# timoklein/alphazero-gym

Measured on NVIDIA B200. Metric: MCTS simulations/sec (batched trees), higher is better.
Workload: dtype f64 tree statistics + env dynamics / f32 network with exact int8-sliced tensor-core products

## Files before the change

### alphazero_gym_b200/csrc/engine.cu

```cuda
#include <cuda_runtime.h>

#include <cmath>
#include <cstdio>
#include <cstdlib>
#include <cstring>
#include <initializer_list>
#include <map>
#include <string>
#include <tuple>
#include <utility>
#include <vector>

#include "../../include/azg.h"
#include "common.cuh"
#include "env.cuh"
#include "mlp.cuh"
#include "qmlp.cuh"
#include "qmlp2.cuh"
#include "search_wg.cuh"
#include "selfplay.cuh"
#include "tree_continuous.cuh"
#include "tree_discrete.cuh"

static thread_local std::string g_err;
// ... 713 lines not shown
            if (ce != cudaSuccess || ee != cudaSuccess) {
                if (g) cudaGraphDestroy(g);
                return fail(AZG_ECUDA, std::string("graph capture: ") + cudaGetErrorString(ce != cudaSuccess ? ce : ee));
            }
            cudaGraphExec_t ge = nullptr;
            cudaError_t ie = cudaGraphInstantiate(&ge, g, 0);
            cudaGraphDestroy(g);
            if (ie != cudaSuccess) return fail(AZG_ECUDA, std::string("graph instantiate: ") + cudaGetErrorString(ie));
            if (e->graphs.size() > 32) {
                for (auto& kv : e->graphs) cudaGraphExecDestroy(kv.second);
                e->graphs.clear();
            }
            e->graphs[key] = ge;
            e->launches = n;
            it = e->graphs.find(key);
        }
        e->launches = 2 * (int64_t)N + 3 + (e->cfg.variant == AZG_CONTINUOUS ? 1 : 0) - (tape ? N + 1 : 0);
        if (e->tree_word != tree_id0) {
            k_set_seed<<<1, 1, 0, st>>>(e->d_seed + 1, (uint64_t)tree_id0);
            CK(cudaGetLastError());
            e->tree_word = tree_id0;
        }
        CK(cudaGraphLaunch(it->second, st));
    }
    e->last_B = B;
    e->last_N = N;
    return AZG_OK;
}

extern "C" int azg_search_discrete(azg_engine* e, int32_t B, const double* d_root_state, const int32_t* d_root_n_init,
                                   int32_t n_rollouts, int64_t tree_id0, void* stream) {
    if (e && e->cfg.variant != AZG_DISCRETE) return fail(AZG_EINVAL, "engine was created for the continuous variant");
    return run_search(e, B, d_root_state, d_root_n_init, n_rollouts, tree_id0, (cudaStream_t)stream);
}

extern "C" int azg_search_continuous(azg_engine* e, int32_t B, const double* d_root_state, int32_t n_rollouts, int64_t tree_id0,
                                     void* stream) {
    if (e && e->cfg.variant != AZG_CONTINUOUS) return fail(AZG_EINVAL, "engine was created for the discrete variant");
    return run_search(e, B, d_root_state, nullptr, n_rollouts, tree_id0, (cudaStream_t)stream);
}

extern "C" int azg_profile_search(azg_engine* e, int32_t B, const double* d_root_state, const int32_t* d_root_n_init,
                                  int32_t n_rollouts, int64_t tree_id0, void* stream, float ms_out[3], int32_t launches_out[3]) {
    if (!e || !d_root_state || !ms_out || !launches_out) return fail(AZG_EINVAL, "null argument");
    if (B < 1 || B > e->cfg.max_trees) return fail(AZG_EINVAL, "B out of range");
    if (n_rollouts < 1 || n_rollouts > e->cfg.max_rollouts) return fail(AZG_EINVAL, "n_rollouts out of range");
    if (!e->weights_set && !e->tapeV) return fail(AZG_EINVAL, "azg_set_weights has not been called");
    CK(cudaSetDevice(e->cfg.device));
    cudaStream_t st = (cudaStream_t)stream;
    const int sd = e->cfg.variant == AZG_DISCRETE ? 4 : 2;
    if (d_root_state != e->root_state)
        CK(cudaMemcpyAsync(e->root_state, d_root_state, (size_t)B * sd * sizeof(double), cudaMemcpyDeviceToDevice, st));
    if (e->cfg.variant == AZG_DISCRETE) {
        if (d_root_n_init) CK(cudaMemcpyAsync(e->root_n_init, d_root_n_init, (size_t)B * sizeof(int32_t), cudaMemcpyDeviceToDevice, st));
        else CK(cudaMemsetAsync(e->root_n_init, 0, (size_t)B * sizeof(int32_t), st));
    }
    Prof prof;
    cudaError_t ce = cudaSuccess;
    e->launches = enqueue_search(e, B, n_rollouts, tree_id0, st, &ce, &prof);
    cudaError_t se = cudaStreamSynchronize(st);
    for (int k = 0; k < 3; ++k) { ms_out[k] = 0.0f; launches_out[k] = 0; }
    for (size_t i = 0; i < prof.cls.size(); ++i) {
        float ms = 0.0f;
        if (cudaEventElapsedTime(&ms, prof.ev[2 * i], prof.ev[2 * i + 1]) == cudaSuccess) {
            ms_out[prof.cls[i]] += ms;
            launches_out[prof.cls[i]] += 1;
        }
    }
    for (cudaEvent_t ev : prof.ev) cudaEventDestroy(ev);
    if (ce != cudaSuccess) return fail(AZG_ECUDA, std::string("kernel launch: ") + cudaGetErrorString(ce));
    if (se != cudaSuccess) return fail(AZG_ECUDA, std::string("sync: ") + cudaGetErrorString(se));
    e->last_B = B;
    e->last_N = n_rollouts;
    return AZG_OK;
}

extern "C" int azg_root_results(azg_engine* e, int32_t B, float* d_actions, int32_t* d_counts, double* d_Q, double* d_V_target,
                                int32_t* d_n_children, void* stream) {
    if (!e || !d_actions || !d_counts || !d_Q || !d_V_target || !d_n_children) return fail(AZG_EINVAL, "null argument");
    if (B < 1 || B > e->cfg.max_trees) return fail(AZG_EINVAL, "B out of range");
    CK(cudaSetDevice(e->cfg.device));
    cudaStream_t st = (cudaStream_t)stream;
    const TreeParams p = make_params(e, B, 0);
    const int tb = 128, tg = (B + tb - 1) / tb;
    if (e->cfg.variant == AZG_DISCRETE) k_results_discrete<<<tg, tb, 0, st>>>(p, e->cmax, d_actions, d_counts, d_Q, d_V_target, d_n_children);
    else k_results_continuous<<<tg, tb, 0, st>>>(p, e->cmax, d_actions, d_counts, d_Q, d_V_target, d_n_children);
    CK(cudaGetLastError());
    return AZG_OK;
}

extern "C" int azg_status(azg_engine* e, void* stream) {
    if (!e) return fail(AZG_EINVAL, "null engine");
    CK(cudaSetDevice(e->cfg.device));
    int32_t h = 0;
    CK(cudaMemcpyAsync(&h, e->err, sizeof h, cudaMemcpyDeviceToHost, (cudaStream_t)stream));
    CK(cudaStreamSynchronize((cudaStream_t)stream));
    if (h) CK(cudaMemsetAsync(e->err, 0, sizeof h, (cudaStream_t)stream));
    if (h & ERR_NAN) return fail(AZG_ENAN, "NaN in a UCT vector (helpers.py:47-48)");
    if (h & ERR_CAPACITY) return fail(AZG_ECAPACITY, "tree arena or child fan-out capacity exceeded");
    return AZG_OK;
}

extern "C" int azg_search_host(azg_engine* e, int32_t B, const double* h_root_state, const int32_t* h_root_n_init, int32_t n_rollouts,
                               int64_t tree_id0, float* h_actions, int32_t* h_counts, double* h_Q, double* h_V_target,
                               int32_t* h_n_children) {
    if (!e || !h_root_state || !h_actions || !h_counts || !h_Q || !h_V_target || !h_n_children) return fail(AZG_EINVAL, "null argument");
    if (B < 1 || B > e->cfg.max_trees) return fail(AZG_EINVAL, "B out of range");
    if (e->cfg.variant == AZG_CONTINUOUS && h_root_n_init) return fail(AZG_EINVAL, "root_n_init is a discrete-only argument");
    CK(cudaSetDevice(e->cfg.device));
    cudaStream_t st = e->own_stream;
    const int sd = e->cfg.variant == AZG_DISCRETE ? 4 : 2;
    const size_t cm = e->cmax;
    char* hp = (char*)e->h_pinned;
    double* p_root = (double*)hp; hp += (size_t)B * 4 * sizeof(double);
    double* p_Q = (double*)hp; hp += (size_t)B * cm * sizeof(double);
    double* p_Vt = (double*)hp; hp += (size_t)B * sizeof(double);
    float* p_act = (float*)hp; hp += (size_t)B * cm * sizeof(float);
    int32_t* p_cnt = (int32_t*)hp; hp += (size_t)B * cm * sizeof(int32_t);
    int32_t* p_nc = (int32_t*)hp; hp += (size_t)B * sizeof(int32_t);
    int32_t* p_rn = (int32_t*)hp;
    {
        cudaPointerAttributes at;
        const bool root_pinned = cudaPointerGetAttributes(&at, h_root_state) == cudaSuccess && at.type == cudaMemoryTypeHost;
        cudaGetLastError();
        if (!root_pinned) memcpy(p_root, h_root_state, (size_t)B * sd * sizeof(double));
        CK(cudaMemcpyAsync(e->root_state, root_pinned ? h_root_state : p_root, (size_t)B * sd * sizeof(double), cudaMemcpyHostToDevice, st));
    }
    const int32_t* d_rn = nullptr;
    if (h_root_n_init) {
        memcpy(p_rn, h_root_n_init, (size_t)B * sizeof(int32_t));
        CK(cudaMemcpyAsync(e->root_n_init, p_rn, (size_t)B * sizeof(int32_t), cudaMemcpyHostToDevice, st));
        d_rn = e->root_n_init;
    }
    int rc = run_search(e, B, e->root_state, d_rn, n_rollouts, tree_id0, st);
    if (rc) return rc;
    rc = azg_root_results(e, B, e->r_actions, e->r_counts, e->r_Q, e->r_Vt, e->r_nchild, st);
    if (rc) return rc;
    auto pinned = [](const void* h) {
        cudaPointerAttributes at;
        const bool ok = cudaPointerGetAttributes(&at, h) == cudaSuccess && at.type == cudaMemoryTypeHost;
        cudaGetLastError();
        return ok;
    };
    const bool direct = pinned(h_actions) && pinned(h_counts) && pinned(h_Q) && pinned(h_V_target) && pinned(h_n_children);
    CK(cudaMemcpyAsync(direct ? h_actions : p_act, e->r_actions, (size_t)B * cm * sizeof(float), cudaMemcpyDeviceToHost, st));
    CK(cudaMemcpyAsync(direct ? h_counts : p_cnt, e->r_counts, (size_t)B * cm * sizeof(int32_t), cudaMemcpyDeviceToHost, st));
    CK(cudaMemcpyAsync(direct ? h_Q : p_Q, e->r_Q, (size_t)B * cm * sizeof(double), cudaMemcpyDeviceToHost, st));
    CK(cudaMemcpyAsync(direct ? h_V_target : p_Vt, e->r_Vt, (size_t)B * sizeof(double), cudaMemcpyDeviceToHost, st));
    CK(cudaMemcpyAsync(direct ? h_n_children : p_nc, e->r_nchild, (size_t)B * sizeof(int32_t), cudaMemcpyDeviceToHost, st));
    rc = azg_status(e, st);
    if (!direct) {
        memcpy(h_actions, p_act, (size_t)B * cm * sizeof(float));
        memcpy(h_counts, p_cnt, (size_t)B * cm * sizeof(int32_t));
        memcpy(h_Q, p_Q, (size_t)B * cm * sizeof(double));
        memcpy(h_V_target, p_Vt, (size_t)B * sizeof(double));
        memcpy(h_n_children, p_nc, (size_t)B * sizeof(int32_t));
    }
    return rc;
}

extern "C" int azg_search_host_begin(azg_engine* e, int32_t slot, int32_t B, const double* h_root_state, const int32_t* h_root_n_init,
                                     int32_t n_rollouts, int64_t tree_id0, float* h_actions, int32_t* h_counts, double* h_Q,
                                     double* h_V_target, int32_t* h_n_children) {
    if (!e || !h_root_state || !h_actions || !h_counts || !h_Q || !h_V_target || !h_n_children) return fail(AZG_EINVAL, "null argument");
    if (slot < 0 || slot > 1) return fail(AZG_EINVAL, "slot must be 0 or 1");
    if (B < 1 || B > e->cfg.max_trees) return fail(AZG_EINVAL, "B out of range");
    if (e->cfg.variant == AZG_CONTINUOUS && h_root_n_init) return fail(AZG_EINVAL, "root_n_init is a discrete-only argument");
    if (e->pending[slot]) return fail(AZG_EINVAL, "slot is still in flight: call azg_search_host_end first");
    CK(cudaSetDevice(e->cfg.device));
    auto pinned = [](const void* h) {
        cudaPointerAttributes at;
        const bool ok = cudaPointerGetAttributes(&at, h) == cudaSuccess && at.type == cudaMemoryTypeHost;
        cudaGetLastError();
        return ok;
    };
    if (!(pinned(h_root_state) && pinned(h_actions) && pinned(h_counts) && pinned(h_Q) && pinned(h_V_target) && pinned(h_n_children) &&
          (!h_root_n_init || pinned(h_root_n_init))))
        return fail(AZG_EINVAL, "azg_search_host_begin needs page-locked host buffers (cudaHostAlloc / cudaHostRegister / pin_memory)");
    const size_t cm = e->cmax, Bm = e->cfg.max_trees;
    if (!e->copy_stream) {
        CK(cudaStreamCreateWithFlags(&e->copy_stream, cudaStreamNonBlocking));
        for (int k = 0; k < 2; ++k) {
            CK(cudaEventCreateWithFlags(&e->ev_done[k], cudaEventDisableTiming));
            CK(cudaEventCreateWithFlags(&e->ev_copied[k], cudaEventDisableTiming));
        }
        CK(cudaMallocHost(&e->h_err, 2 * sizeof(int32_t)));
        CK(cudaMalloc(&e->r2_actions, Bm * cm * sizeof(float)));
        CK(cudaMalloc(&e->r2_counts, Bm * cm * sizeof(int32_t)));
        CK(cudaMalloc(&e->r2_Q, Bm * cm * sizeof(double)));
        CK(cudaMalloc(&e->r2_Vt, Bm * sizeof(double)));
        CK(cudaMalloc(&e->r2_nchild, Bm * sizeof(int32_t)));
    }
    float* ra = slot ? e->r2_actions : e->r_actions;
    int32_t* rc_ = slot ? e->r2_counts : e->r_counts;
    double* rq = slot ? e->r2_Q : e->r_Q;
    double* rv = slot ? e->r2_Vt : e->r_Vt;
    int32_t* rn = slot ? e->r2_nchild : e->r_nchild;
    cudaStream_t st = e->own_stream;
    const int sd = e->cfg.variant == AZG_DISCRETE ? 4 : 2;
    CK(cudaMemcpyAsync(e->root_state, h_root_state, (size_t)B * sd * sizeof(double), cudaMemcpyHostToDevice, st));
    const int32_t* d_rn = nullptr;
    if (h_root_n_init) {
        CK(cudaMemcpyAsync(e->root_n_init, h_root_n_init, (size_t)B * sizeof(int32_t), cudaMemcpyHostToDevice, st));
        d_rn = e->root_n_init;
    }
    int rc = run_search(e, B, e->root_state, d_rn, n_rollouts, tree_id0, st);
    if (rc) return rc;
    rc = azg_root_results(e, B, ra, rc_, rq, rv, rn, st);
    if (rc) return rc;
    CK(cudaMemcpyAsync(e->h_err + slot, e->err, sizeof(int32_t), cudaMemcpyDeviceToHost, st));
    CK(cudaMemsetAsync(e->err, 0, sizeof(int32_t), st));
    CK(cudaEventRecord(e->ev_done[slot], st));
    CK(cudaStreamWaitEvent(e->copy_stream, e->ev_done[slot], 0));
    CK(cudaMemcpyAsync(h_actions, ra, (size_t)B * cm * sizeof(float), cudaMemcpyDeviceToHost, e->copy_stream));
    CK(cudaMemcpyAsync(h_counts, rc_, (size_t)B * cm * sizeof(int32_t), cudaMemcpyDeviceToHost, e->copy_stream));
    CK(cudaMemcpyAsync(h_Q, rq, (size_t)B * cm * sizeof(double), cudaMemcpyDeviceToHost, e->copy_stream));
    CK(cudaMemcpyAsync(h_V_target, rv, (size_t)B * sizeof(double), cudaMemcpyDeviceToHost, e->copy_stream));
    CK(cudaMemcpyAsync(h_n_children, rn, (size_t)B * sizeof(int32_t), cudaMemcpyDeviceToHost, e->copy_stream));
    CK(cudaEventRecord(e->ev_copied[slot], e->copy_stream));
    e->pending[slot] = true;
    return AZG_OK;
}

extern "C" int azg_search_host_end(azg_engine* e, int32_t slot) {
    if (!e || slot < 0 || slot > 1) return fail(AZG_EINVAL, "bad argument");
    if (!e->pending[slot]) return fail(AZG_EINVAL, "nothing in flight in this slot");
    CK(cudaSetDevice(e->cfg.device));
    CK(cudaEventSynchronize(e->ev_copied[slot]));
    e->pending[slot] = false;
    const int32_t h = e->h_err[slot];
    if (h & ERR_NAN) return fail(AZG_ENAN, "NaN in a UCT vector (helpers.py:47-48)");
    if (h & ERR_CAPACITY) return fail(AZG_ECAPACITY, "tree arena or child fan-out capacity exceeded");
    return AZG_OK;
}

static cudaError_t fetch_ctl(const azg_engine* e, int B, std::vector<CCtl>& out) {
    const size_t BS = e->cfg.max_trees;
    std::vector<uint4> plane(B);
    out.resize(B);
    for (int k = 0; k < 4; ++k) {
        cudaError_t ce = cudaMemcpy(plane.data(), e->ctl + k * BS, (size_t)B * sizeof(uint4), cudaMemcpyDeviceToHost);
        if (ce != cudaSuccess) return ce;
        for (int t = 0; t < B; ++t) reinterpret_cast<uint4*>(&out[t])[k] = plane[t];
    }
    return cudaSuccess;
}
static cudaError_t fetch_et(const azg_engine* e, int B, std::vector<CHot>& out) {
    const size_t BS = e->cfg.max_trees;
    std::vector<CHot> plane(B);
    out.resize((size_t)B * CROOT_MAX_KIDS);
    for (int j = 0; j < CROOT_MAX_KIDS; ++j) {
        cudaError_t ce = cudaMemcpy(plane.data(), e->et + j * BS, (size_t)B * sizeof(CHot), cudaMemcpyDeviceToHost);
        if (ce != cudaSuccess) return ce;
        for (int t = 0; t < B; ++t) out[(size_t)t * CROOT_MAX_KIDS + j] = plane[t];
    }
    return cudaSuccess;
}

extern "C" int azg_get_counters(azg_engine* e, int32_t B, int64_t out[8]) {
    if (!e || !out) return fail(AZG_EINVAL, "null argument");
    if (B < 1 || B > e->cfg.max_trees) return fail(AZG_EINVAL, "B out of range");
    CK(cudaSetDevice(e->cfg.device));
    CK(cudaDeviceSynchronize());
    std::vector<uint32_t> c(4 * (size_t)B);
    std::vector<int32_t> dr(B, 0), pw(B, 0);
    const int LB = e->last_B > 0 ? e->last_B : B;
    std::vector<uint32_t> all(4 * (size_t)LB);
    CK(cudaMemcpy(all.data(), e->ctr, all.size() * sizeof(uint32_t), cudaMemcpyDeviceToHost));
    if (e->cfg.variant == AZG_DISCRETE) {
        CK(cudaMemcpy(dr.data(), e->draws, (size_t)B * sizeof(int32_t), cudaMemcpyDeviceToHost));
    } else {
        std::vector<CCtl> cc;
        CK(fetch_ctl(e, B, cc));
        for (int t = 0; t < B; ++t) { dr[t] = cc[t].draws; pw[t] = cc[t].pw; }
    }
    for (int k = 0; k < 8; ++k) out[k] = 0;
    const int nb = std::min(B, LB);
    for (int t = 0; t < nb; ++t) {
        out[1] += all[t];
        out[2] += all[(size_t)LB + t];
        out[6] += all[(size_t)2 * LB + t];
        out[4] += all[(size_t)3 * LB + t];
        out[5] += dr[t];
        out[3] += pw[t];
    }
    out[0] = (int64_t)nb * e->last_N;
    out[7] = e->launches;
    return AZG_OK;
}

extern "C" int azg_fused_stats(azg_engine* e, int64_t out[8]) {
    if (!e || !out) return fail(AZG_EINVAL, "null argument");
    CK(cudaSetDevice(e->cfg.device));
    CK(cudaDeviceSynchronize());
    unsigned long long h[16];
    CK(cudaMemcpy(h, e->stats, sizeof h, cudaMemcpyDeviceToHost));
    CK(cudaMemset(e->stats, 0, sizeof h));
#ifdef AZG_TREE_PROF
    fprintf(stderr, "tree step sections (cycles summed over warps): load %llu backup %llu select %llu insert %llu expand+store %llu | per-WG total %llu over %llu warpgroups | "
            "discrete level loop: scores %llu draw+pick %llu next row %llu over %llu warp-levels\n", h[8], h[9], h[10], h[11], h[12], h[0], h[4], h[13], h[14], h[11], h[15]);
#endif
#ifdef AZG_EVAL_PROF
    if (e->last_fused_kind == 2)
        fprintf(stderr, "k_search_wg, cycles per warpgroup and search spent waiting for MMAs: at column step 0 of a layer %llu | step 1 %llu | steps 2..7 %llu | kernel %llu\n",
                h[8] / (h[4] ? h[4] : 1), h[9] / (h[4] ? h[4] : 1), h[10] / (h[4] ? h[4] : 1), h[0] / (h[4] ? h[4] : 1));
    else
    fprintf(stderr, "evaluation timeline of epilogue thread 0, cycles per CTA and search: layer 0 %llu | MMA wait %llu | load + convert %llu | stash / quantise / heads %llu | "
            "post-processing wait %llu | tree phase %llu | kernel %llu\n", h[8] / (h[4] ? h[4] : 1), h[9] / (h[4] ? h[4] : 1), h[10] / (h[4] ? h[4] : 1), h[11] / (h[4] ? h[4] : 1),
            h[12] / (h[4] ? h[4] : 1), h[13] / (h[4] ? h[4] : 1), h[0] / (h[4] ? h[4] : 1));
#endif
    for (int k = 0; k < 8; ++k) out[k] = (int64_t)h[k];
    out[5] = e->last_fused_kind;
    return AZG_OK;
}

extern "C" int azg_set_seed(azg_engine* e, uint64_t seed, void* stream) {
    if (!e) return fail(AZG_EINVAL, "null engine");
    CK(cudaSetDevice(e->cfg.device));
    k_set_seed<<<1, 1, 0, (cudaStream_t)stream>>>(e->d_seed, seed);
    CK(cudaGetLastError());
    e->cfg.seed = seed;
    return AZG_OK;
}

extern "C" int azg_set_reward_model(azg_engine* e, double reward_step, double reward_terminal) {
    if (!e) return fail(AZG_EINVAL, "null engine");
    if (!(reward_step == reward_step) || !(reward_terminal == reward_terminal) || std::isinf(reward_step) || std::isinf(reward_terminal))
        return fail(AZG_EINVAL, "rewards must be finite");
    if (e->cfg.variant != AZG_DISCRETE && (reward_step != 1.0 || reward_terminal != 1.0))
        return fail(AZG_EINVAL, "the reward model applies to the discrete (CartPole) search");
    if (reward_step == e->reward_step && reward_terminal == e->reward_terminal) return AZG_OK;
    CK(cudaSetDevice(e->cfg.device));
    CK(cudaDeviceSynchronize());
    for (auto& kv : e->graphs) cudaGraphExecDestroy(kv.second);
    e->graphs.clear();
    e->reward_step = reward_step; e->reward_terminal = reward_terminal;
    return AZG_OK;
}

extern "C" uint64_t azg_selfplay_seed(uint64_t seed, int64_t step_index) { return seed + (uint64_t)step_index * 0x9E3779B97F4A7C15ull; }

extern "C" int azg_selfplay_step(azg_engine* e, int32_t B, const azg_selfplay_io* io, int32_t n_rollouts, int64_t tree_id0,
                                 int64_t step_index, uint64_t base_seed, int32_t max_episode_length, int32_t deterministic,
                                 int32_t by_value, double temperature, void* stream) {
    if (!e || !io) return fail(AZG_EINVAL, "null argument");
    if (!io->d_env_state || !io->d_ep_step || !io->d_episode || !io->d_obs || !io->d_actions || !io->d_counts || !io->d_Q ||
        !io->d_V_target || !io->d_n_children || !io->d_action_taken || !io->d_reward || !io->d_done)
        return fail(AZG_EINVAL, "null buffer in azg_selfplay_io");
    const bool disc = e->cfg.variant == AZG_DISCRETE;
    if (disc && !io->d_root_n) return fail(AZG_EINVAL, "d_root_n is required for the discrete variant");
    if (max_episode_length < 1) return fail(AZG_EINVAL, "max_episode_length must be >= 1");
    if (!(temperature > 0.0)) return fail(AZG_EINVAL, "temperature must be > 0");
    cudaStream_t st = (cudaStream_t)stream;
    int rc = azg_set_seed(e, azg_selfplay_seed(base_seed, step_index), stream);
    if (rc) return rc;
    rc = run_search(e, B, io->d_env_state, disc ? io->d_root_n : nullptr, n_rollouts, tree_id0, st);
    if (rc) return rc;
    rc = azg_root_results(e, B, io->d_actions, io->d_counts, io->d_Q, io->d_V_target, io->d_n_children, stream);
    if (rc) return rc;
    SelfPlayParams sp;
    memset(&sp, 0, sizeof sp);
    sp.B = B; sp.cmax = e->cmax; sp.max_episode_length = max_episode_length; sp.deterministic = deterministic; sp.by_value = by_value;
    sp.temperature = temperature; sp.tree_id0 = tree_id0; sp.seedp = e->d_seed;
    sp.env_state = io->d_env_state; sp.ep_step = io->d_ep_step; sp.episode = io->d_episode; sp.root_n = io->d_root_n;
    sp.actions = io->d_actions; sp.counts = io->d_counts; sp.Q = io->d_Q; sp.n_children = io->d_n_children;
    sp.obs = io->d_obs; sp.action_taken = io->d_action_taken; sp.reward = io->d_reward; sp.done = io->d_done;
    sp.drows = e->drows; sp.R = e->R;
    const int tb = 128, tg = (B + tb - 1) / tb;
    if (disc) k_selfplay_discrete<<<tg, tb, 0, st>>>(sp);
    else k_selfplay_continuous<<<tg, tb, 0, st>>>(sp);
    CK(cudaGetLastError());
    return AZG_OK;
}

extern "C" int azg_dump_tree_discrete(azg_engine* e, int32_t B, const azg_dump_discrete* o) {
    if (!e || !o) return fail(AZG_EINVAL, "null argument");
    if (e->cfg.variant != AZG_DISCRETE) return fail(AZG_EINVAL, "engine is not discrete");
    if (B < 1 || B > e->cfg.max_trees) return fail(AZG_EINVAL, "B out of range");
    CK(cudaSetDevice(e->cfg.device));
    CK(cudaDeviceSynchronize());
    const size_t R = e->R, A = 2;
    std::vector<DRow> rows((size_t)B * R);
    std::vector<double> st((size_t)B * R * 4);
    std::vector<int32_t> nr(B);
    CK(cudaMemcpy(rows.data(), e->drows, rows.size() * sizeof(DRow), cudaMemcpyDeviceToHost));
    CK(cudaMemcpy(st.data(), e->dstate, st.size() * sizeof(double), cudaMemcpyDeviceToHost));
    CK(cudaMemcpy(nr.data(), e->n_rows, (size_t)B * sizeof(int32_t), cudaMemcpyDeviceToHost));
    for (size_t t = 0; t < (size_t)B; ++t) {
        o->n_nodes[t] = nr[t];
        for (size_t i = 0; i < R; ++i) {
            const size_t q = t * R + i;
            const bool live = (int)i < nr[t];
            const DRow& r = rows[q];
            o->parent[q] = live ? (r.parent == DROW_NONE ? -1 : r.parent) : 0;
            o->paction[q] = live ? (r.parent == DROW_NONE ? -1 : r.paction) : 0;
            o->node_n[q] = live ? r.node_n : 0;
            o->terminal[q] = live ? (r.flags & ROW_TERMINAL) : 0;
            o->V[q] = live ? r.V : 0.0f;
            o->r[q] = live ? r.r : 0.0;
            for (size_t k = 0; k < 4; ++k) o->state[q * 4 + k] = live ? st[q * 4 + k] : 0.0;
            for (size_t a = 0; a < A; ++a) {
                o->prior[q * A + a] = live ? r.prior[a] : 0.0f;
                o->eW[q * A + a] = live ? r.W[a] : 0.0;
                o->en[q * A + a] = live ? r.n_e[a] : 0;
                o->echild[q * A + a] = live ? (r.child[a] == DROW_NONE ? -1 : r.child[a]) : 0;
            }
        }
    }
    return AZG_OK;
}

extern "C" int azg_dump_tree_continuous(azg_engine* e, int32_t B, const azg_dump_continuous* o) {
    if (!e || !o) return fail(AZG_EINVAL, "null argument");
    if (e->cfg.variant != AZG_CONTINUOUS) return fail(AZG_EINVAL, "engine is not continuous");
    if (B < 1 || B > e->cfg.max_trees) return fail(AZG_EINVAL, "B out of range");
    CK(cudaSetDevice(e->cfg.device));
    CK(cudaDeviceSynchronize());
    const size_t R = e->R, K3 = e->K3, HS = e->HS;
    std::vector<CRow> rows((size_t)B * R);
    std::vector<CHot> et;
    std::vector<CCtl> ctl;
    std::vector<float> hd((size_t)B * R * HS);
    CK(cudaMemcpy(rows.data(), e->crows, rows.size() * sizeof(CRow), cudaMemcpyDeviceToHost));
    CK(fetch_et(e, B, et));
    CK(fetch_ctl(e, B, ctl));
    CK(cudaMemcpy(hd.data(), e->chead, hd.size() * sizeof(float), cudaMemcpyDeviceToHost));
    std::vector<int32_t> par(R);
    std::vector<const CHot*> hot(R);
    for (size_t t = 0; t < (size_t)B; ++t) {
        const int nr = ctl[t].n_rows;
        o->n_rows[t] = nr;
        for (size_t i = 0; i < R; ++i) { par[i] = -1; hot[i] = reinterpret_cast<const CHot*>(&rows[t * R + i]); }
        for (int k = 0; k < ctl[t].root_nk && k < CROOT_MAX_KIDS; ++k) {
            const size_t kid = ctl[t].root_kids[k];
            if (kid < R) { par[kid] = 0; hot[kid] = &et[t * CROOT_MAX_KIDS + k]; }
        }
        for (size_t i = 1; i < R && (int)i < nr; ++i) {
            if (!(hot[i]->nn_flags & CROW_EXPANDED)) continue;
            const CRow& r = rows[t * R + i];
            for (int k = 0; k < r.nkids && k < CROW_MAX_KIDS; ++k)
                if (r.kids[k] < R) par[r.kids[k]] = (int32_t)i;
        }
        for (size_t i = 0; i < R; ++i) {
            const size_t q = t * R + i;
            const bool live = (int)i < nr;
            const CHot& h = *hot[i];
            const CRow& r = rows[q];
            const bool ex = live && (h.nn_flags & CROW_EXPANDED);
            o->parent[q] = live ? par[i] : 0;
            o->action[q] = live && i > 0 ? h.action : 0.0f;
            o->eW[q] = live ? h.W : 0.0;
            o->en[q] = live ? h.n_e : 0;
            o->expanded[q] = ex ? 1 : 0;
            o->node_n[q] = ex ? (i == 0 ? ctl[t].root_nn : (int32_t)(h.nn_flags & CROW_NMASK)) : 0;
            o->terminal[q] = ex && (h.nn_flags & CROW_TERMINAL) ? 1 : 0;
            o->V[q] = ex ? h.V : 0.0f;
            o->r[q] = ex ? h.r : 0.0;
            o->state[q * 2] = ex ? r.th : 0.0;
            o->state[q * 2 + 1] = ex ? r.thdot : 0.0;
            for (size_t k = 0; k < K3; ++k) o->head[q * K3 + k] = ex ? hd[q * HS + k] : 0.0f;
        }
    }
    return AZG_OK;
}

extern "C" int azg_mlp_forward(azg_engine* e, int32_t n, const float* d_x, float* d_V, float* d_head, void* stream) {
    if (!e || !d_x || !d_V || !d_head) return fail(AZG_EINVAL, "null argument");
    if (n < 1) return fail(AZG_EINVAL, "n must be >= 1");
    if (!e->weights_set) return fail(AZG_EINVAL, "azg_set_weights has not been called");
    CK(cudaSetDevice(e->cfg.device));
    MlpParams m = make_mlp_params(e, n);
    m.X = d_x; m.xstride = e->cfg.state_dim; m.mode = 1; m.outV = d_V; m.outHead = d_head; m.evals = nullptr;
    CK(launch_mlp(e, m, (cudaStream_t)stream, false));
    return AZG_OK;
}

__global__ void k_env_step(int variant, int n, const double* s, const float* a, double* o, double* rew, int32_t* term, float* obs) {
    const int i = blockIdx.x * blockDim.x + threadIdx.x;
    if (i >= n) return;
    if (variant == AZG_DISCRETE) {
        const double in[4] = {s[i * 4], s[i * 4 + 1], s[i * 4 + 2], s[i * 4 + 3]};
        double out[4], r;
        const bool t = env::cartpole_step(in, (int)a[i], out, r);
        for (int k = 0; k < 4; ++k) { o[i * 4 + k] = out[k]; obs[i * 4 + k] = (float)out[k]; }
        rew[i] = r;
        term[i] = t;
    } else {
        double nth, nthdot, r;
        const bool t = env::pendulum_step(s[i * 2], s[i * 2 + 1], a[i], nth, nthdot, r);
        o[i * 2] = nth; o[i * 2 + 1] = nthdot;
        const float4 ob = env::pendulum_obs(nth, nthdot);
        obs[i * 3] = ob.x; obs[i * 3 + 1] = ob.y; obs[i * 3 + 2] = ob.z;
        rew[i] = r;
        term[i] = t;
    }
}

extern "C" int azg_env_step(azg_engine* e, int32_t n, const double* d_state, const float* d_action, double* d_next, double* d_reward,
                            int32_t* d_terminal, float* d_obs, void* stream) {
    if (!e || !d_state || !d_action || !d_next || !d_reward || !d_terminal || !d_obs) return fail(AZG_EINVAL, "null argument");
    if (n < 1) return fail(AZG_EINVAL, "n must be >= 1");
    CK(cudaSetDevice(e->cfg.device));
    k_env_step<<<(n + 127) / 128, 128, 0, (cudaStream_t)stream>>>(e->cfg.variant, n, d_state, d_action, d_next, d_reward, d_terminal, d_obs);
    CK(cudaGetLastError());
    return AZG_OK;
}
```

### alphazero_gym_b200/csrc/search_wg.cuh

```cuda
#pragma once
#include "qmlp2.cuh"

#define WG_THREADS 640
#define WG_EPI_THREADS 512
#define WG_IDESC(N) ((2u << 4) | (1u << 7) | (1u << 10) | (((uint32_t)(N) >> 3) << 17) | ((128u >> 4) << 24))
#define WG_B_KCHUNK 6144
#define WG_B_STEP 768
#define WG_WIN_COLS 48
#define WG_STASH_COL 96
#define WG_SLOT_COLS 224
#define WG_MAX_ROUNDS 4

__host__ __device__ inline size_t search_wg_smem_bytes(int NL, int qfl_count) {
    return (size_t)NL * 3 * QMLP_PLANE + 2 * 3 * QMLP_PLANE + (size_t)qfl_count * 4 + 1024 + Q2_TAB_BYTES;
}

__device__ __forceinline__ void umma_i8_wg(uint32_t tmem_d, uint32_t da_lo, uint32_t db_lo, uint32_t idesc, uint32_t accumulate) {
    asm volatile(
        "{\n\t.reg .pred p;\n\t.reg .b64 da, db;\n\tmov.b64 da, {%1, %5};\n\tmov.b64 db, {%2, %5};\n\tsetp.ne.b32 p, %4, 0;\n\t"
        "tcgen05.mma.cta_group::1.kind::i8 [%0], da, db, %3, p;\n\t}" ::"r"(tmem_d),
        "r"(da_lo), "r"(db_lo), "r"(idesc), "r"(accumulate), "r"(Q2_DESC_HI)
        : "memory");
}
__device__ __forceinline__ uint32_t wg_descb_lo(uint32_t saddr) { return ((saddr >> 4) & 0x3FFFu) | (((uint32_t)WG_B_KCHUNK >> 4) << 16); }

#ifndef WG_EPI_REGS
#define WG_EPI_REGS 104
#define WG_MMA_REGS 56
#endif

__device__ __forceinline__ void mbar_arrive_s(uint32_t bar) { asm volatile("mbarrier.arrive.shared::cta.b64 _, [%0];" ::"r"(bar) : "memory"); }
__device__ __forceinline__ bool mbar_try_wait_s(uint32_t bar, uint32_t parity, uint32_t ns) {
    uint32_t ok;
    asm volatile("{\n\t.reg .pred p;\n\tmbarrier.try_wait.parity.shared::cta.b64 p, [%1], %2, %3;\n\tselp.u32 %0, 1, 0, p;\n\t}"
                 : "=r"(ok) : "r"(bar), "r"(parity), "r"(ns) : "memory");
    return ok != 0;
}
__device__ __forceinline__ void mbar_wait_s(uint32_t bar, uint32_t parity) {
    int spins = 0;
    while (!mbar_try_wait_s(bar, parity, 20000u)) {
        if (++spins > (1 << 22)) {
            printf("mbar_wait timeout: block %d thread %d barrier smem 0x%x parity %u\n", blockIdx.x, threadIdx.x, bar, parity);
            __trap();
        }
    }
}

struct WgSlot {
    uint32_t tacc;
    int8_t* sA;
    uint32_t ready, full, accfree, slotfree;
    uint32_t fullph;
    long long cyc_full;
#ifdef AZG_EVAL_PROF
    long long cyc_k[3];
#endif
};

__device__ __forceinline__ float wg_quantise_row(const WgSlot& sl, bool wact, int r, float pm) {
    float cx = 0.0f;
    if (wact) {
        const int e = q8_exponent(pm);
        const float sx = __uint_as_float((uint32_t)(276 - e) << 23);
        cx = __uint_as_float((uint32_t)(e - 22) << 23);
#pragma unroll 2
        for (int c = 0; c < 8; ++c) {
            float v[16];
            tmem_ld16f(sl.tacc + WG_STASH_COL + 16 * c, v);
            tmem_wait_ld();
            q8_store16(v, sx, sl.sA, c, r);
        }
        asm volatile("fence.proxy.async.shared::cta;" ::: "memory");
    }
    tc_fence_before();
    mbar_arrive_s(sl.ready);
    return cx;
}

template <int S, int ACT, int NL>
__device__ __forceinline__ void wg_evaluate(const MlpParams& p, WgSlot& sl, const float* fl, bool wact, bool valid, int gr, int r, float* out) {
    const float* W0 = fl;
    const float* b0 = fl + S * 128;
    const float2* cwb = reinterpret_cast<const float2*>(fl + S * 128 + 128);
    const float* Wh = fl + S * 128 + 128 + NL * 2 * 128;
    const float* bh = Wh + 128 * p.PO_PAD;
    float pm = 0.0f;
    if (wact) {
        float x[S];
#pragma unroll
        for (int s = 0; s < S; ++s) x[s] = 0.0f;
        if (valid) {
            const float4 v = *reinterpret_cast<const float4*>(p.X + (size_t)gr * 4);
            x[0] = v.x; x[1] = v.y; x[2] = v.z;
            if (S > 3) x[S - 1] = v.w;
        }
#pragma unroll 1
        for (int c = 0; c < 8; ++c) {
            float a[16];
#pragma unroll
            for (int i = 0; i < 16; i += 2) {
                const int j = c * 16 + i;
                float2 acc = *reinterpret_cast<const float2*>(b0 + j);
#pragma unroll
                for (int s = 0; s < S; ++s) acc = __ffma2_rn(make_float2(x[s], x[s]), *reinterpret_cast<const float2*>(W0 + s * 128 + j), acc);
                const float2 e = mlp_act2<ACT>(acc);
                a[i] = e.x; a[i + 1] = e.y;
                pm = fmaxf(pm, fmaxf(fabsf(e.x), fabsf(e.y)));
            }
            tmem_st16f(sl.tacc + WG_STASH_COL + 16 * c, a);
        }
        tmem_wait_st();
    }
    float cx = wg_quantise_row(sl, wact, r, pm);
#pragma unroll 1
    for (int l = 0; l < NL; ++l) {
        pm = 0.0f;
#pragma unroll 1
        for (int k = 0; k < 8; ++k) {
            const int w = k & 1;
            const long long f0 = clock64();
            mbar_wait_s(sl.full + 8u * w, (sl.fullph >> w) & 1u);
            sl.fullph ^= 1u << w;
            tc_fence_after();
            sl.cyc_full += clock64() - f0;
#ifdef AZG_EVAL_PROF
            sl.cyc_k[k < 2 ? k : 2] += clock64() - f0;
#endif
            if (wact) {
                const uint32_t ta = sl.tacc + w * WG_WIN_COLS;
                int32_t pa[16], pb[16], pc[16];
                tmem_ld16(ta, pa);
                tmem_ld16(ta + 16, pb);
                tmem_ld16(ta + 32, pc);
                tmem_wait_ld();
                tc_fence_before();
                if (k < 6) mbar_arrive_s(sl.accfree + 8u * w);
                const float2* cb = cwb + l * 128 + 16 * k;
                float v[16];
#pragma unroll
                for (int i = 0; i < 16; i += 2) {
                    const float4 sb = *reinterpret_cast<const float4*>(cb + i);
                    float u0 = __int2float_rn(pa[i] * 256 + pb[i]);
                    float u1 = __int2float_rn(pa[i + 1] * 256 + pb[i + 1]);
                    u0 = __fmaf_rn(u0, 256.0f, q8_i2f_23(pc[i]));
                    u1 = __fmaf_rn(u1, 256.0f, q8_i2f_23(pc[i + 1]));
                    const float2 y = make_float2(__fmaf_rn(u0, __fmul_rn(cx, sb.x), sb.y), __fmaf_rn(u1, __fmul_rn(cx, sb.z), sb.w));
                    const float2 ev = mlp_act2<ACT>(y);
                    v[i] = ev.x; v[i + 1] = ev.y;
                    pm = fmaxf(pm, fmaxf(fabsf(ev.x), fabsf(ev.y)));
                }
                tmem_st16f(sl.tacc + WG_STASH_COL + 16 * k, v);
            } else {
                tc_fence_before();
                if (k < 6) mbar_arrive_s(sl.accfree + 8u * w);
            }
        }
        if (wact) tmem_wait_st();
        if (l + 1 < NL) cx = wg_quantise_row(sl, wact, r, pm);
    }
    if (wact) {
#pragma unroll 1
        for (int c4 = 0; c4 < p.PO_PAD / 4; ++c4) {
            float2 lo[4], hi[4];
#pragma unroll
            for (int q = 0; q < 4; ++q) {
                lo[q] = make_float2(0.0f, 0.0f);
                hi[q] = make_float2(0.0f, 0.0f);
#pragma unroll
                for (int hc = 0; hc < 2; ++hc) {
                    float a[16];
                    tmem_ld16f(sl.tacc + WG_STASH_COL + 32 * q + 16 * hc, a);
                    tmem_wait_ld();
                    const float* wp = Wh + (32 * q + 16 * hc) * p.PO_PAD + c4 * 4;
#pragma unroll
                    for (int i = 0; i < 16; ++i) {
                        const float4 w4 = *reinterpret_cast<const float4*>(wp + i * p.PO_PAD);
                        const float2 av = make_float2(a[i], a[i]);
                        lo[q] = __ffma2_rn(av, make_float2(w4.x, w4.y), lo[q]);
                        hi[q] = __ffma2_rn(av, make_float2(w4.z, w4.w), hi[q]);
                    }
                }
            }
            const float s0 = __fadd_rn(__fadd_rn(__fadd_rn(lo[0].x, lo[1].x), __fadd_rn(lo[2].x, lo[3].x)), bh[c4 * 4 + 0]);
            const float s1 = __fadd_rn(__fadd_rn(__fadd_rn(lo[0].y, lo[1].y), __fadd_rn(lo[2].y, lo[3].y)), bh[c4 * 4 + 1]);
            const float s2 = __fadd_rn(__fadd_rn(__fadd_rn(hi[0].x, hi[1].x), __fadd_rn(hi[2].x, hi[3].x)), bh[c4 * 4 + 2]);
            const float s3 = __fadd_rn(__fadd_rn(__fadd_rn(hi[0].y, hi[1].y), __fadd_rn(hi[2].y, hi[3].y)), bh[c4 * 4 + 3]);
#pragma unroll
            for (int g4 = 0; g4 < Q2_MAX_PO / 4; ++g4)
                if (g4 == c4) { out[4 * g4] = s0; out[4 * g4 + 1] = s1; out[4 * g4 + 2] = s2; out[4 * g4 + 3] = s3; }
        }
    }
    tc_fence_before();
}

template <int S, int ACT, int NL>
__global__ void __launch_bounds__(WG_THREADS, 1)
k_search_wg(const MlpParams p, const TreeParams tp, const int n_sims, const int chunk_begin, const int chunk_end) {
    extern __shared__ __align__(1024) uint8_t wsm_raw[];
    __shared__ __align__(8) uint64_t wbar, ready[2], full[2][2], accfree[2][2], slotfree[2][2];
    __shared__ uint32_t tmem_base_s;
    uint8_t* qsm = wsm_raw + ((1024u - (smem_u32(wsm_raw) & 1023u)) & 1023u);
    int8_t* sB = reinterpret_cast<int8_t*>(qsm);
    int8_t* sA = sB + (size_t)NL * 3 * QMLP_PLANE;
    float* fl = reinterpret_cast<float*>(sA + 2 * 3 * QMLP_PLANE);
    double* s_rcp = reinterpret_cast<double*>(fl + p.qfl_count);
    double* s_sq = s_rcp + FUSED_TAB + 1;
    int32_t* s_pw = reinterpret_cast<int32_t*>(s_sq + FUSED_TAB + 1);

    const int tid = threadIdx.x, warp = tid >> 5, lane = tid & 31;
    const int per = (chunk_end - chunk_begin + gridDim.x - 1) / gridDim.x;
    const int row_begin = chunk_begin + blockIdx.x * per;
    const int row_end = min(row_begin + per, chunk_end);
    if (row_begin >= row_end) return;
    const int nrows = row_end - row_begin;
    const int rounds = (nrows + 511) / 512;
    const int ntiles_max = 4 * rounds;
    int th = (nrows + ntiles_max - 1) / ntiles_max;
    if (th > 32) th = (th + 31) & ~31;
    const int ntiles = (nrows + th - 1) / th;
    const int n_evals = n_sims + 1;

    if (tid == 0) {
        mbar_init(&wbar, 1);
        for (int s = 0; s < 2; ++s) {
            mbar_init(&ready[s], 128);
            mbar_init(&slotfree[s][0], 128);
            mbar_init(&slotfree[s][1], 128);
            for (int w = 0; w < 2; ++w) {
                mbar_init(&full[s][w], 1);
                mbar_init(&accfree[s][w], 128);
            }
        }
    }
    if (warp == 0) {
        asm volatile("tcgen05.alloc.cta_group::1.sync.aligned.shared::cta.b32 [%0], %1;" ::"r"(smem_u32(&tmem_base_s)), "n"(512) : "memory");
        asm volatile("tcgen05.relinquish_alloc_permit.cta_group::1.sync.aligned;" ::: "memory");
    }
    tc_fence_before();
    __syncthreads();
    tc_fence_after();
    const uint32_t tb = tmem_base_s;
#ifdef AZG_WG_DEBUG
    if (tid == 0 && blockIdx.x == 0)
        printf("wg: wbar 0x%x ready 0x%x full 0x%x accfree 0x%x slotfree 0x%x tmem 0x%x nrows %d th %d ntiles %d rounds %d\n", smem_u32(&wbar), smem_u32(ready),
               smem_u32(&full[0][0]), smem_u32(&accfree[0][0]), smem_u32(&slotfree[0][0]), tb, nrows, th, ntiles, rounds);
#endif
    if (tid == 0) {
        const uint32_t bytesB = (uint32_t)NL * 3 * QMLP_PLANE, bytesF = (uint32_t)p.qfl_count * 4u;
        mbar_expect_tx(&wbar, bytesB + bytesF);
        for (uint32_t o = 0; o < bytesB; o += 32768u) bulk_g2s(sB + o, p.qdigits_nat + o, min(32768u, bytesB - o), &wbar);
        bulk_g2s(fl, p.qfl, bytesF, &wbar);
    }
    for (int i = tid; i <= FUSED_TAB; i += blockDim.x) {
        s_rcp[i] = tp.rcp_tab[i];
        s_sq[i] = tp.sqrt_tab[i];
        s_pw[i] = (tp.pw_table && i < p.R) ? tp.pw_table[i] : 0;
    }
    __syncthreads();
    mbar_wait(&wbar, 0);

    if (warp >= 16) {
        asm volatile("setmaxnreg.dec.sync.aligned.u32 %0;" ::"n"(WG_MMA_REGS));
        if (warp < 18) {
            const int slot = warp - 16;
            uint32_t rph = 0, aph = 0;
            const uint32_t aH = q2_desc_lo(smem_u32(sA) + (uint32_t)slot * 3 * QMLP_PLANE), aM = aH + 1024, aL = aH + 2048;
#pragma unroll 1
            for (int s = 0; s < n_evals; ++s)
#pragma unroll 1
            for (int rd = 0; rd < rounds; ++rd)
#pragma unroll 1
            for (int half = 0; half < 2; ++half) {
                if (4 * rd + slot + 2 * half >= ntiles) continue;
#pragma unroll 1
                for (int l = 0; l < NL; ++l) {
#pragma unroll 1
                    for (int k = 0; k < 8; ++k) {
                        const int w = k & 1;
                        if (k == 0) { mbar_wait(&ready[slot], rph); rph ^= 1u; }
                        else if (k >= 2) { mbar_wait(&accfree[slot][w], (aph >> w) & 1u); aph ^= 1u << w; }
                        tc_fence_after();
                        const uint32_t bq = wg_descb_lo(smem_u32(sB) + (uint32_t)l * 3 * QMLP_PLANE + (uint32_t)k * WG_B_STEP);
                        const uint32_t acc = tb + slot * WG_SLOT_COLS + w * WG_WIN_COLS;
                        if (elect_one()) {
#pragma unroll
                        for (int kk = 0; kk < 4; ++kk) {
                            umma_i8_wg(acc, aH + kk * 256, bq + kk * 768, WG_IDESC(48), kk > 0);
                            umma_i8_wg(acc + 16, aM + kk * 256, bq + kk * 768, WG_IDESC(32), 1);
                            umma_i8_wg(acc + 32, aL + kk * 256, bq + kk * 768, WG_IDESC(16), 1);
                        }
                        umma_commit(&full[slot][w]);
                        }
                        __syncwarp();
                    }
                }
            }
        }
    } else {
        asm volatile("setmaxnreg.inc.sync.aligned.u32 %0;" ::"n"(WG_EPI_REGS));
        const int g = warp >> 2, slot = g & 1, half = g >> 1;
        const int r = (warp & 3) * 32 + lane;
        WgSlot sl;
        sl.tacc = tb + ((uint32_t)((warp & 3) * 32) << 16) + slot * WG_SLOT_COLS;
        sl.sA = sA + (size_t)slot * 3 * QMLP_PLANE;
        sl.ready = smem_u32(&ready[slot]); sl.full = smem_u32(full[slot]); sl.accfree = smem_u32(accfree[slot]); sl.slotfree = smem_u32(slotfree[slot]);
        sl.fullph = 0;
        sl.cyc_full = 0;
#ifdef AZG_EVAL_PROF
        sl.cyc_k[0] = sl.cyc_k[1] = sl.cyc_k[2] = 0;
#endif
        bool first_use = true;
        uint32_t useph = 0;
        const Tabs tabs = {s_pw, s_rcp, s_sq, FUSED_TAB};
        long long cyc_tree = 0, cyc_slot = 0;
        const long long cyc_begin = clock64();
        uint32_t nev = 0;
        int ev_row = 0;
        for (int rd = 0; rd < rounds; ++rd) {
            const int tile = 4 * rd + g, row0 = row_begin + tile * th;
            if (tile < ntiles && row0 + r < min(row0 + th, row_end)) {
                if (S == 4) d_init(tp, row0 + r);
                else c_init(tp, row0 + r);
            }
        }
#pragma unroll 1
        for (int s = 0; s < n_evals; ++s) {
#pragma unroll 1
        for (int rd = 0; rd < rounds; ++rd) {
            const int tile = 4 * rd + g;
            const bool tvalid = tile < ntiles;
            const int row0 = row_begin + tile * th;
            const int nv = tvalid ? max(0, min(th, row_end - row0)) : 0;
            const int gr = row0 + r;
            const bool valid = r < nv, wact = (warp & 3) * 32 < nv;
            const long long c0 = clock64();
            if (half == 1 || !first_use) {
                mbar_wait_s(sl.slotfree + 8u * (half ^ 1), useph);
                useph ^= 1u;
            }
            first_use = false;
            tc_fence_after();
            const long long c1 = clock64();
            float out[Q2_MAX_PO];
#pragma unroll
            for (int i = 0; i < Q2_MAX_PO; ++i) out[i] = 0.0f;
            if (tvalid) wg_evaluate<S, ACT, NL>(p, sl, fl, wact, valid, gr, r, out);
            mbar_arrive_s(sl.slotfree + 8u * half);
            const long long c2 = clock64();
            if (valid) {
                int leafw;
                double lr = 0.0;
                if (p.variant == 1) {
                    const uint4 k0 = p.ctl[gr], k1 = p.ctl[(size_t)p.BS + gr];
                    leafw = (int)k0.z;
                    lr = __hiloint2double((int)k1.w, (int)k1.z);
                } else {
                    leafw = p.leaf[gr];
                }
                if (leafw & LEAF_EVAL) {
                    mlp_finish_row(p, gr, leafw, lr, out[0], out + 1);
                    ++nev;
                    ev_row = gr;
                }
                if (S == 4) {
                    d_step(tp, tabs, gr, s > 0, s + 1 < n_evals);
                } else {
                    if (s == 0) c_root_insert(tp, gr);
                    c_step(tp, tabs, gr, s > 0, s + 1 < n_evals);
                }
            }
            cyc_slot += c1 - c0;
            cyc_tree += clock64() - c2;
        }
        }
        if (nev) p.evals[ev_row] += nev;
        if ((warp & 3) == 0 && lane == 0 && p.stats) {
            atomicAdd(p.stats + 0, (unsigned long long)(clock64() - cyc_begin));
            atomicAdd(p.stats + 1, (unsigned long long)cyc_tree);
            atomicAdd(p.stats + 2, (unsigned long long)cyc_slot);
            atomicAdd(p.stats + 3, (unsigned long long)sl.cyc_full);
#ifdef AZG_EVAL_PROF
            for (int k = 0; k < 3; ++k) atomicAdd(p.stats + 8 + k, (unsigned long long)sl.cyc_k[k]);
#endif
            atomicAdd(p.stats + 4, 1ull);
        }
    }
    tc_fence_before();
    __syncthreads();
    if (warp == 0) asm volatile("tcgen05.dealloc.cta_group::1.sync.aligned.b32 %0, %1;" ::"r"(tb), "n"(512) : "memory");
}
```

Before: 1.146 billion.

## Double-buffer TMEM loads in quantise and heads, pack epilogue math into float2 FMAs

Several epilogue micro-optimisations land together. The quantise loop and the output-head loop now issue the next TMEM load before processing the current one, overlapping load latency with compute. Heads are specialised on a compile-time PO so their loops unroll fully. The dequantise/bias step uses paired float2 FMAs, with the column-scale/bias table reordered once at kernel start to match. The input row load is moved ahead of the slot wait, and mbarrier poll counters are added under the profiling flag. Extra live registers under the fixed epilogue register cap could cause spills.

```diff
diff --git a/alphazero_gym_b200/csrc/engine.cu b/alphazero_gym_b200/csrc/engine.cu
--- a/alphazero_gym_b200/csrc/engine.cu
+++ b/alphazero_gym_b200/csrc/engine.cu
@@ -1039,8 +1039,9 @@
 #endif
 #ifdef AZG_EVAL_PROF
     if (e->last_fused_kind == 2)
-        fprintf(stderr, "k_search_wg, cycles per warpgroup and search spent waiting for MMAs: at column step 0 of a layer %llu | step 1 %llu | steps 2..7 %llu | kernel %llu\n",
-                h[8] / (h[4] ? h[4] : 1), h[9] / (h[4] ? h[4] : 1), h[10] / (h[4] ? h[4] : 1), h[0] / (h[4] ? h[4] : 1));
+        fprintf(stderr, "k_search_wg, cycles per warpgroup and search spent waiting for MMAs: at column step 0 of a layer %llu | step 1 %llu | steps 2..7 %llu | kernel %llu | "
+                "mbarrier polls per warp and search: MMA waits %llu | slot waits %llu\n",
+                h[8] / (h[4] ? h[4] : 1), h[9] / (h[4] ? h[4] : 1), h[10] / (h[4] ? h[4] : 1), h[0] / (h[4] ? h[4] : 1), h[11] / (h[4] ? h[4] : 1), h[12] / (h[4] ? h[4] : 1));
     else
     fprintf(stderr, "evaluation timeline of epilogue thread 0, cycles per CTA and search: layer 0 %llu | MMA wait %llu | load + convert %llu | stash / quantise / heads %llu | "
             "post-processing wait %llu | tree phase %llu | kernel %llu\n", h[8] / (h[4] ? h[4] : 1), h[9] / (h[4] ? h[4] : 1), h[10] / (h[4] ? h[4] : 1), h[11] / (h[4] ? h[4] : 1),
diff --git a/alphazero_gym_b200/csrc/search_wg.cuh b/alphazero_gym_b200/csrc/search_wg.cuh
--- a/alphazero_gym_b200/csrc/search_wg.cuh
+++ b/alphazero_gym_b200/csrc/search_wg.cuh
@@ -36,14 +36,15 @@
                  : "=r"(ok) : "r"(bar), "r"(parity), "r"(ns) : "memory");
     return ok != 0;
 }
-__device__ __forceinline__ void mbar_wait_s(uint32_t bar, uint32_t parity) {
-    int spins = 0;
+__device__ __forceinline__ uint32_t mbar_wait_s(uint32_t bar, uint32_t parity) {
+    uint32_t spins = 1;
     while (!mbar_try_wait_s(bar, parity, 20000u)) {
-        if (++spins > (1 << 22)) {
+        if (++spins > (1u << 22)) {
             printf("mbar_wait timeout: block %d thread %d barrier smem 0x%x parity %u\n", blockIdx.x, threadIdx.x, bar, parity);
             __trap();
         }
     }
+    return spins;
 }
 
 struct WgSlot {
@@ -54,6 +55,7 @@
     long long cyc_full;
 #ifdef AZG_EVAL_PROF
     long long cyc_k[3];
+    long long polls_full, polls_slot;
 #endif
 };
 
@@ -63,12 +65,17 @@
         const int e = q8_exponent(pm);
         const float sx = __uint_as_float((uint32_t)(276 - e) << 23);
         cx = __uint_as_float((uint32_t)(e - 22) << 23);
-#pragma unroll 2
-        for (int c = 0; c < 8; ++c) {
-            float v[16];
-            tmem_ld16f(sl.tacc + WG_STASH_COL + 16 * c, v);
+        float v0[16], v1[16];
+        tmem_ld16f(sl.tacc + WG_STASH_COL, v0);
+        tmem_wait_ld();
+#pragma unroll 1
+        for (int c = 0; c < 8; c += 2) {
+            tmem_ld16f(sl.tacc + WG_STASH_COL + 16 * (c + 1), v1);
+            q8_store16(v0, sx, sl.sA, c, r);
             tmem_wait_ld();
-            q8_store16(v, sx, sl.sA, c, r);
+            if (c + 2 < 8) tmem_ld16f(sl.tacc + WG_STASH_COL + 16 * (c + 2), v0);
+            q8_store16(v1, sx, sl.sA, c + 1, r);
+            tmem_wait_ld();
         }
         asm volatile("fence.proxy.async.shared::cta;" ::: "memory");
     }
@@ -77,23 +84,52 @@
     return cx;
 }
 
+template <int PO>
+__device__ __forceinline__ void wg_heads(const WgSlot& sl, const float* Wh, float* out) {
+    const float* bh = Wh + 128 * PO;
+#pragma unroll 1
+    for (int c4 = 0; c4 < PO / 4; ++c4) {
+        float2 lo[4], hi[4];
+#pragma unroll
+        for (int q = 0; q < 4; ++q) lo[q] = hi[q] = make_float2(0.0f, 0.0f);
+        float a[2][16];
+        tmem_ld16f(sl.tacc + WG_STASH_COL, a[0]);
+        tmem_wait_ld();
+#pragma unroll
+        for (int j = 0; j < 8; ++j) {
+            const int q = j >> 1;
+            if (j + 1 < 8) tmem_ld16f(sl.tacc + WG_STASH_COL + 16 * (j + 1), a[(j + 1) & 1]);
+            const float* wp = Wh + 16 * j * PO + c4 * 4;
+#pragma unroll
+            for (int i = 0; i < 16; ++i) {
+                const float4 w4 = *reinterpret_cast<const float4*>(wp + i * PO);
+                const float2 av = make_float2(a[j & 1][i], a[j & 1][i]);
+                lo[q] = __ffma2_rn(av, make_float2(w4.x, w4.y), lo[q]);
+                hi[q] = __ffma2_rn(av, make_float2(w4.z, w4.w), hi[q]);
+            }
+            if (j + 1 < 8) tmem_wait_ld();
+        }
+        const float s0 = __fadd_rn(__fadd_rn(__fadd_rn(lo[0].x, lo[1].x), __fadd_rn(lo[2].x, lo[3].x)), bh[c4 * 4 + 0]);
+        const float s1 = __fadd_rn(__fadd_rn(__fadd_rn(lo[0].y, lo[1].y), __fadd_rn(lo[2].y, lo[3].y)), bh[c4 * 4 + 1]);
+        const float s2 = __fadd_rn(__fadd_rn(__fadd_rn(hi[0].x, hi[1].x), __fadd_rn(hi[2].x, hi[3].x)), bh[c4 * 4 + 2]);
+        const float s3 = __fadd_rn(__fadd_rn(__fadd_rn(hi[0].y, hi[1].y), __fadd_rn(hi[2].y, hi[3].y)), bh[c4 * 4 + 3]);
+#pragma unroll
+        for (int g4 = 0; g4 < Q2_MAX_PO / 4; ++g4)
+            if (g4 == c4) { out[4 * g4] = s0; out[4 * g4 + 1] = s1; out[4 * g4 + 2] = s2; out[4 * g4 + 3] = s3; }
+    }
+}
+
 template <int S, int ACT, int NL>
-__device__ __forceinline__ void wg_evaluate(const MlpParams& p, WgSlot& sl, const float* fl, bool wact, bool valid, int gr, int r, float* out) {
+__device__ __forceinline__ void wg_evaluate(const MlpParams& p, WgSlot& sl, const float* fl, bool wact, float4 v, int r, float* out) {
     const float* W0 = fl;
     const float* b0 = fl + S * 128;
     const float2* cwb = reinterpret_cast<const float2*>(fl + S * 128 + 128);
     const float* Wh = fl + S * 128 + 128 + NL * 2 * 128;
-    const float* bh = Wh + 128 * p.PO_PAD;
     float pm = 0.0f;
     if (wact) {
         float x[S];
-#pragma unroll
-        for (int s = 0; s < S; ++s) x[s] = 0.0f;
-        if (valid) {
-            const float4 v = *reinterpret_cast<const float4*>(p.X + (size_t)gr * 4);
-            x[0] = v.x; x[1] = v.y; x[2] = v.z;
-            if (S > 3) x[S - 1] = v.w;
-        }
+        x[0] = v.x; x[1] = v.y; x[2] = v.z;
+        if (S > 3) x[S - 1] = v.w;
 #pragma unroll 1
         for (int c = 0; c < 8; ++c) {
             float a[16];
@@ -119,12 +155,15 @@
         for (int k = 0; k < 8; ++k) {
             const int w = k & 1;
             const long long f0 = clock64();
-            mbar_wait_s(sl.full + 8u * w, (sl.fullph >> w) & 1u);
+            const uint32_t np = mbar_wait_s(sl.full + 8u * w, (sl.fullph >> w) & 1u);
             sl.fullph ^= 1u << w;
             tc_fence_after();
             sl.cyc_full += clock64() - f0;
 #ifdef AZG_EVAL_PROF
             sl.cyc_k[k < 2 ? k : 2] += clock64() - f0;
+            sl.polls_full += np;
+#else
+            (void)np;
 #endif
             if (wact) {
                 const uint32_t ta = sl.tacc + w * WG_WIN_COLS;
@@ -137,14 +176,13 @@
                 if (k < 6) mbar_arrive_s(sl.accfree + 8u * w);
                 const float2* cb = cwb + l * 128 + 16 * k;
                 float v[16];
+                const float2 cx2 = make_float2(cx, cx);
 #pragma unroll
                 for (int i = 0; i < 16; i += 2) {
                     const float4 sb = *reinterpret_cast<const float4*>(cb + i);
-                    float u0 = __int2float_rn(pa[i] * 256 + pb[i]);
-                    float u1 = __int2float_rn(pa[i + 1] * 256 + pb[i + 1]);
-                    u0 = __fmaf_rn(u0, 256.0f, q8_i2f_23(pc[i]));
-                    u1 = __fmaf_rn(u1, 256.0f, q8_i2f_23(pc[i + 1]));
-                    const float2 y = make_float2(__fmaf_rn(u0, __fmul_rn(cx, sb.x), sb.y), __fmaf_rn(u1, __fmul_rn(cx, sb.z), sb.w));
+                    float2 u = make_float2(__int2float_rn(pa[i] * 256 + pb[i]), __int2float_rn(pa[i + 1] * 256 + pb[i + 1]));
+                    u = __ffma2_rn(u, make_float2(256.0f, 256.0f), make_float2(q8_i2f_23(pc[i]), q8_i2f_23(pc[i + 1])));
+                    const float2 y = __ffma2_rn(u, __fmul2_rn(cx2, make_float2(sb.x, sb.y)), make_float2(sb.z, sb.w));
                     const float2 ev = mlp_act2<ACT>(y);
                     v[i] = ev.x; v[i + 1] = ev.y;
                     pm = fmaxf(pm, fmaxf(fabsf(ev.x), fabsf(ev.y)));
@@ -159,35 +197,11 @@
         if (l + 1 < NL) cx = wg_quantise_row(sl, wact, r, pm);
     }
     if (wact) {
-#pragma unroll 1
-        for (int c4 = 0; c4 < p.PO_PAD / 4; ++c4) {
-            float2 lo[4], hi[4];
-#pragma unroll
-            for (int q = 0; q < 4; ++q) {
-                lo[q] = make_float2(0.0f, 0.0f);
-                hi[q] = make_float2(0.0f, 0.0f);
-#pragma unroll
-                for (int hc = 0; hc < 2; ++hc) {
-                    float a[16];
-                    tmem_ld16f(sl.tacc + WG_STASH_COL + 32 * q + 16 * hc, a);
-                    tmem_wait_ld();
-                    const float* wp = Wh + (32 * q + 16 * hc) * p.PO_PAD + c4 * 4;
-#pragma unroll
-                    for (int i = 0; i < 16; ++i) {
-                        const float4 w4 = *reinterpret_cast<const float4*>(wp + i * p.PO_PAD);
-                        const float2 av = make_float2(a[i], a[i]);
-                        lo[q] = __ffma2_rn(av, make_float2(w4.x, w4.y), lo[q]);
-                        hi[q] = __ffma2_rn(av, make_float2(w4.z, w4.w), hi[q]);
-                    }
-                }
-            }
-            const float s0 = __fadd_rn(__fadd_rn(__fadd_rn(lo[0].x, lo[1].x), __fadd_rn(lo[2].x, lo[3].x)), bh[c4 * 4 + 0]);
-            const float s1 = __fadd_rn(__fadd_rn(__fadd_rn(lo[0].y, lo[1].y), __fadd_rn(lo[2].y, lo[3].y)), bh[c4 * 4 + 1]);
-            const float s2 = __fadd_rn(__fadd_rn(__fadd_rn(hi[0].x, hi[1].x), __fadd_rn(hi[2].x, hi[3].x)), bh[c4 * 4 + 2]);
-            const float s3 = __fadd_rn(__fadd_rn(__fadd_rn(hi[0].y, hi[1].y), __fadd_rn(hi[2].y, hi[3].y)), bh[c4 * 4 + 3]);
-#pragma unroll
-            for (int g4 = 0; g4 < Q2_MAX_PO / 4; ++g4)
-                if (g4 == c4) { out[4 * g4] = s0; out[4 * g4 + 1] = s1; out[4 * g4 + 2] = s2; out[4 * g4 + 3] = s3; }
+        switch (p.PO_PAD) {
+            case 4: wg_heads<4>(sl, Wh, out); break;
+            case 8: wg_heads<8>(sl, Wh, out); break;
+            case 12: wg_heads<12>(sl, Wh, out); break;
+            default: wg_heads<16>(sl, Wh, out); break;
         }
     }
     tc_fence_before();
@@ -258,6 +272,14 @@
     }
     __syncthreads();
     mbar_wait(&wbar, 0);
+    {
+        float4* cw4 = reinterpret_cast<float4*>(fl + S * 128 + 128);
+        for (int i = tid; i < NL * 64; i += blockDim.x) {
+            const float4 t = cw4[i];
+            cw4[i] = make_float4(t.x, t.z, t.y, t.w);
+        }
+        __syncthreads();
+    }
 
     if (warp >= 16) {
         asm volatile("setmaxnreg.dec.sync.aligned.u32 %0;" ::"n"(WG_MMA_REGS));
@@ -308,6 +330,7 @@
         sl.cyc_full = 0;
 #ifdef AZG_EVAL_PROF
         sl.cyc_k[0] = sl.cyc_k[1] = sl.cyc_k[2] = 0;
+        sl.polls_full = sl.polls_slot = 0;
 #endif
         bool first_use = true;
         uint32_t useph = 0;
@@ -333,9 +356,16 @@
             const int nv = tvalid ? max(0, min(th, row_end - row0)) : 0;
             const int gr = row0 + r;
             const bool valid = r < nv, wact = (warp & 3) * 32 < nv;
+            float4 xin = make_float4(0.0f, 0.0f, 0.0f, 0.0f);
+            if (valid) xin = *reinterpret_cast<const float4*>(p.X + (size_t)gr * 4);
             const long long c0 = clock64();
             if (half == 1 || !first_use) {
-                mbar_wait_s(sl.slotfree + 8u * (half ^ 1), useph);
+                const uint32_t np = mbar_wait_s(sl.slotfree + 8u * (half ^ 1), useph);
+#ifdef AZG_EVAL_PROF
+                sl.polls_slot += np;
+#else
+                (void)np;
+#endif
                 useph ^= 1u;
             }
             first_use = false;
@@ -344,7 +374,7 @@
             float out[Q2_MAX_PO];
 #pragma unroll
             for (int i = 0; i < Q2_MAX_PO; ++i) out[i] = 0.0f;
-            if (tvalid) wg_evaluate<S, ACT, NL>(p, sl, fl, wact, valid, gr, r, out);
+            if (tvalid) wg_evaluate<S, ACT, NL>(p, sl, fl, wact, xin, r, out);
             mbar_arrive_s(sl.slotfree + 8u * half);
             const long long c2 = clock64();
             if (valid) {
@@ -381,6 +411,8 @@
             atomicAdd(p.stats + 3, (unsigned long long)sl.cyc_full);
 #ifdef AZG_EVAL_PROF
             for (int k = 0; k < 3; ++k) atomicAdd(p.stats + 8 + k, (unsigned long long)sl.cyc_k[k]);
+            atomicAdd(p.stats + 11, (unsigned long long)sl.polls_full);
+            atomicAdd(p.stats + 12, (unsigned long long)sl.polls_slot);
 #endif
             atomicAdd(p.stats + 4, 1ull);
         }
```

After: 1.174 billion, median of 6. 2.4% higher.
